# yangao07/longcallD

Measured on AMD Instinct MI355X. Metric: regions_per_sec, higher is better.
Workload: dtype int32; 1 GPU; configs[1]: synthetic 30x hifi region jobs, 10 Mb of reference per step (1250 regions/step, ~20.2 Mbase POA-aligned/step); distinct_batches_per_gpu=32, warmup_on_other_seeds=True, lanes_per_gpu=2

## Files before the change

longcalld_amd/csrc/edlib_kernel.hip:

```cpp
#include <hip/hip_runtime.h>
#include "lcd_types.h"
#include "lcd_kernels.h"

namespace {

typedef unsigned long long Word;

__device__ __forceinline__ int imin(int a, int b) { return a < b ? a : b; }
__device__ __forceinline__ int wave_shr1(const int v) { return __builtin_amdgcn_update_dpp(0, v, 0x138, 0xf, 0xf, false); }

__device__ __forceinline__ int calc_block(Word Pv, Word Mv, Word Eq, int hin, Word &PvOut, Word &MvOut) {
    const Word hinIsNeg = (Word)(hin < 0);
    const Word Xv = Eq | Mv;
    Eq |= hinIsNeg;
    const Word Xh = (((Eq & Pv) + Pv) ^ Pv) | Eq;
    Word Ph = Mv | ~(Xh | Pv);
    Word Mh = Pv & Xh;
    int hout = (int)(Ph >> 63) - (int)(Mh >> 63);
    Ph <<= 1; Mh <<= 1;
    Mh |= hinIsNeg;
    Ph |= (Word)(hin > 0);
    PvOut = Mh | ~(Xv | Ph);
    MvOut = Ph & Xv;
    return hout;
}

struct Sub {
    const uint8_t *q, *t;
    int qlen, tlen;
};

template <bool STORE, bool COLS>
__device__ __forceinline__ int myers_pass(const Sub &sp, int ncols, bool rev, int lane, Word *P, Word *M, int *S, int *col_out, signed char *hcarry,
                                          unsigned long long *blocks_acc) {
    const int qlen = sp.qlen, nb = (qlen + 63) >> 6;
    int result = 0;
    __shared__ uint8_t tbuf[128];
    for (int tile0 = 0; tile0 < nb; tile0 += 64) {
        const int b = tile0 + lane;
        const bool act = b < nb;
        Word peq[5] = {0, 0, 0, 0, 0};
        if (act) {
            const int base = b << 6, lim = imin(64, qlen - base);
            for (int r = 0; r < lim; ++r) {
                const int qi = base + r;
                const uint8_t c = rev ? sp.q[qlen - 1 - qi] : sp.q[qi];
                const Word bit = 1ull << r;
                if (c == 0) peq[0] |= bit; else if (c == 1) peq[1] |= bit; else if (c == 2) peq[2] |= bit;
                else if (c == 3) peq[3] |= bit; else peq[4] |= bit;
            }
        }
        Word Pv = ~0ull, Mv = 0;
        int score = (b + 1) << 6, hout = 0;
        const bool more = tile0 + 64 < nb;
        const int nsteps = ncols + 63;
        auto tchar = [&](const int cc) -> uint8_t { return cc < ncols ? (rev ? sp.t[sp.tlen - 1 - cc] : sp.t[cc]) : (uint8_t)4; };
        uint8_t tnext = tchar(lane);
        int hcnext = (tile0 != 0 && lane < ncols) ? (int)hcarry[lane] : 0, hcreg = 0;
        for (int step = 0; step < nsteps; ++step) {
            if ((step & 63) == 0) {
                const int cc = step + lane;
                __syncthreads();
                tbuf[cc & 127] = tnext;
                hcreg = hcnext;
                __syncthreads();
                tnext = tchar(cc + 64);
                if (tile0 != 0) hcnext = cc + 64 < ncols ? (int)hcarry[cc + 64] : 0;
            }
            const int hleft = wave_shr1(hout);
            const int c = step - lane;
            const int hc0 = __builtin_amdgcn_readlane(hcreg, step & 63);
            if (act && c >= 0 && c < ncols) {
                const int hin = lane == 0 ? (tile0 == 0 ? 1 : hc0) : hleft;
                const uint8_t tc = tbuf[c & 127];
                const Word Eq = tc == 0 ? peq[0] : tc == 1 ? peq[1] : tc == 2 ? peq[2] : tc == 3 ? peq[3] : peq[4];
                hout = calc_block(Pv, Mv, Eq, hin, Pv, Mv);
                score += hout;
                if (STORE) { const size_t o = (size_t)c * nb + b; P[o] = Pv; M[o] = Mv; S[o] = score; }
                if (more && lane == 63) hcarry[ncols + c] = (signed char)hout;
            }
        }
        __syncthreads();
        if (more) {
            for (int c = lane; c < ncols; c += 64) hcarry[c] = hcarry[ncols + c];
            __syncthreads();
        }
        *blocks_acc += (unsigned long long)ncols * (unsigned long long)(imin(64, nb - tile0));
        if (act) {
            const int base = b << 6, lim = imin(64, qlen - base);
            if (COLS)
                for (int pos = 0; pos < lim; ++pos) {
                    int v = score;
                    if (pos < 63) v += -__popcll(Pv >> (pos + 1)) + __popcll(Mv >> (pos + 1));
                    col_out[base + pos] = v;
                }
        }
        const int lastb = nb - 1;
        if (lastb >= tile0 && lastb < tile0 + 64) {
            const int pos = (qlen - 1) & 63;
            int v = score;
            if (pos < 63) v += -__popcll(Pv >> (pos + 1)) + __popcll(Mv >> (pos + 1));
            result = __shfl(v, lastb - tile0);
        }
        __syncthreads();
    }
    return result;
}

template <int HIN0>
__device__ __forceinline__ void sg_pass(const Sub &sp, int ncols, bool rev, int lane, signed char *hcarry, unsigned long long *blocks_acc, int *best_out, int *first_out, int *last_out) {
    const int qlen = sp.qlen, nb = (qlen + 63) >> 6;
    int best = 1 << 30, first_c = -1, last_c = -1;
    __shared__ uint8_t tbuf2[128];
    for (int tile0 = 0; tile0 < nb; tile0 += 64) {
        const int b = tile0 + lane;
        const bool act = b < nb;
        Word peq[5] = {0, 0, 0, 0, 0};
        if (act) {
            const int base = b << 6, lim = imin(64, qlen - base);
            for (int r = 0; r < lim; ++r) {
                const int qi = base + r;
                const uint8_t c = rev ? sp.q[qlen - 1 - qi] : sp.q[qi];
                const Word bit = 1ull << r;
                if (c == 0) peq[0] |= bit; else if (c == 1) peq[1] |= bit; else if (c == 2) peq[2] |= bit;
                else if (c == 3) peq[3] |= bit; else peq[4] |= bit;
            }
        }
        Word Pv = ~0ull, Mv = 0;
        int score = (b + 1) << 6, hout = 0;
        const bool more = tile0 + 64 < nb;
        const bool is_last = b == nb - 1;
        const int pos = (qlen - 1) & 63;
        const int nsteps = ncols + 63;
        auto tchar = [&](const int cc) -> uint8_t { return cc < ncols ? (rev ? sp.t[sp.tlen - 1 - cc] : sp.t[cc]) : (uint8_t)4; };
        uint8_t tnext = tchar(lane);
        int hcnext = (tile0 != 0 && lane < ncols) ? (int)hcarry[lane] : 0, hcreg = 0;
        for (int step = 0; step < nsteps; ++step) {
            if ((step & 63) == 0) {
                const int cc = step + lane;
                __syncthreads();
                tbuf2[cc & 127] = tnext;
                hcreg = hcnext;
                __syncthreads();
                tnext = tchar(cc + 64);
                if (tile0 != 0) hcnext = cc + 64 < ncols ? (int)hcarry[cc + 64] : 0;
            }
            const int hleft = wave_shr1(hout);
            const int c = step - lane;
            const int hc0 = __builtin_amdgcn_readlane(hcreg, step & 63);
            if (act && c >= 0 && c < ncols) {
                const int hin = lane == 0 ? (tile0 == 0 ? HIN0 : hc0) : hleft;
                const uint8_t tc = tbuf2[c & 127];
                const Word Eq = tc == 0 ? peq[0] : tc == 1 ? peq[1] : tc == 2 ? peq[2] : tc == 3 ? peq[3] : peq[4];
                hout = calc_block(Pv, Mv, Eq, hin, Pv, Mv);
                score += hout;
                if (more && lane == 63) hcarry[ncols + c] = (signed char)hout;
                if (is_last) {
                    int v = score;
                    if (pos < 63) v += -__popcll(Pv >> (pos + 1)) + __popcll(Mv >> (pos + 1));
                    if (v < best) { best = v; first_c = c; last_c = c; } else if (v == best) last_c = c;
                }
            }
        }
        __syncthreads();
        if (more) {
            for (int c = lane; c < ncols; c += 64) hcarry[c] = hcarry[ncols + c];
            __syncthreads();
        }
        *blocks_acc += (unsigned long long)ncols * (unsigned long long)(imin(64, nb - tile0));
        const int lastb = nb - 1;
        if (lastb >= tile0 && lastb < tile0 + 64) { best = __shfl(best, lastb - tile0); first_c = __shfl(first_c, lastb - tile0); last_c = __shfl(last_c, lastb - tile0); }
        __syncthreads();
    }
    *best_out = best; *first_out = first_c; *last_out = last_c;
}

struct Tally {
    int n_mis, n_eq, n_ins, n_del, runs;
    int last_op;
};

}

__global__ void __launch_bounds__(64) lcd_edlib_kernel(const EdJob *jobs, const uint8_t *pool, uint8_t *arena, EdOut *outs, int n_jobs) {
    const int jid = blockIdx.x;
    if (jid >= n_jobs) return;
    const int lane = threadIdx.x;
    const EdJob jb = jobs[jid];
    EdOut out; out.status = LCD_OK; out.dist = -1; out.xgaps = 0; out.n_eq = 0; out.n_xid = 0; out.blocks = 0; out.start = 0; out.end = jb.tlen - 1;
    const uint8_t *q = pool + jb.q_off, *t = pool + jb.t_off;
    const int qlen = jb.qlen, tlen = jb.tlen;
    if (qlen == 0 || tlen == 0) {
        out.dist = jb.mode == 1 ? qlen : (qlen > tlen ? qlen : tlen);
        if (jb.mode == 1) { out.start = -1; out.end = -1; }
        if (lane == 0) outs[jb.pad_] = out;
        return;
    }
    const size_t TB_CAP = (size_t)ed_tb_cap(qlen, tlen);
    uint8_t *ws = arena + jb.ws_off;
    Word *P = (Word *)ws, *M = P + TB_CAP;
    int *S = (int *)(M + TB_CAP);
    int *colL = S + TB_CAP, *colR = colL + qlen;
    signed char *hcarry = (signed char *)(colR + qlen);
    unsigned long long blocks = 0;
    Sub top = {q, t, qlen, tlen};
    int dist, t0 = 0, tl0 = tlen;
    const bool top_leaf = jb.mode != 1 && 20ll * ((qlen + 63) >> 6) * tlen + 8ll * tlen < 1024 * 1024;
    if (jb.mode == 1) {
        int best, endf, endl, best2, sf, sl;
        sg_pass<0>(top, tlen, false, lane, hcarry, &blocks, &best, &endf, &endl);
        if (best >= qlen) {
            out.dist = qlen; out.start = 0; out.end = -1;
            out.xgaps = 1; out.n_eq = 0; out.n_xid = qlen; out.blocks = blocks;
            if (lane == 0) outs[jb.pad_] = out;
            return;
        }
        Sub pre = {q, t, qlen, endf + 1};
        sg_pass<1>(pre, endf + 1, true, lane, hcarry, &blocks, &best2, &sf, &sl);
        if (best2 != best || endf < 0 || sl < 0) { out.status = LCD_ERR_BACKTRACK; if (lane == 0) outs[jb.pad_] = out; return; }
        dist = best; t0 = endf - sl; tl0 = sl + 1;
        out.start = t0; out.end = endf;
    } else if (top_leaf)
        dist = -1;
    else
        dist = myers_pass<false, false>(top, tlen, false, lane, nullptr, nullptr, nullptr, nullptr, hcarry, &blocks);
    out.dist = dist;
    __shared__ int stk[64][5];
    int sp = 0;
    if (lane == 0) { stk[0][0] = 0; stk[0][1] = qlen; stk[0][2] = t0; stk[0][3] = tl0; stk[0][4] = dist; }
    sp = 1;
    __syncthreads();
    Tally T = {0, 0, 0, 0, 0, -1};
    while (sp > 0 && out.status == LCD_OK) {
        --sp;
        const int qo = stk[sp][0], ql = stk[sp][1], to = stk[sp][2], tl = stk[sp][3], best = stk[sp][4];
        __syncthreads();
        if (ql == 0 || tl == 0) {
            const int n = ql + tl;
            if (n > 0) {
                const int op = ql == 0 ? 2 : 1;
                if (op == 2) T.n_del += n; else T.n_ins += n;
                if (T.last_op != op) T.runs++;
                T.last_op = op;
            }
            continue;
        }
        Sub s = {q + qo, t + to, ql, tl};
        const long long nb = (ql + 63) >> 6;
        const long long data_size = 20ll * nb * tl + 8ll * tl;
        if (data_size < 1024 * 1024) {
            const int leaf_score = myers_pass<true, false>(s, tl, false, lane, P, M, S, nullptr, hcarry, &blocks);
            if (top_leaf) out.dist = leaf_score;
            __syncthreads();
            int r_mis = 0, r_eq = 0, r_ins = 0, r_del = 0, r_runs = 0, leaf_first = -1, leaf_last = -1;
            {
                const int NB = (int)nb;
                int c0 = -1, bA = -1;
                Word cPa = 0, cMa = 0, cPb = 0, cMb = 0; int cSa = 0, cSb = 0;
                auto refresh = [&](const int r, const int c) {
                    c0 = c; bA = r >> 6;
                    const int cl = c - lane;
                    if (cl >= 0) {
                        const size_t oa = (size_t)cl * NB + bA;
                        cPa = P[oa]; cMa = M[oa]; cSa = S[oa];
                        if (bA > 0) { cPb = P[oa - 1]; cMb = M[oa - 1]; cSb = S[oa - 1]; }
                    }
                };
                auto rl64 = [&](const Word v, const int l) { return (Word)(unsigned)__builtin_amdgcn_readlane((int)(unsigned)v, l) | ((Word)(unsigned)__builtin_amdgcn_readlane((int)(unsigned)(v >> 32), l) << 32); };
                auto val = [&](const int r, const int c) -> int {
                    if (r < 0) return c + 1;
                    if (c < 0) return r + 1;
                    const int b = r >> 6, l = __builtin_amdgcn_readfirstlane(c0 - c), pos = r & 63;
                    Word pv, mv; int sv;
                    if (l >= 0 && l < 64 && b == bA) { pv = rl64(cPa, l); mv = rl64(cMa, l); sv = __builtin_amdgcn_readlane(cSa, l); }
                    else if (l >= 0 && l < 64 && b == bA - 1) { pv = rl64(cPb, l); mv = rl64(cMb, l); sv = __builtin_amdgcn_readlane(cSb, l); }
                    else { const size_t o = (size_t)c * NB + b; pv = P[o]; mv = M[o]; sv = S[o]; }
                    return sv + (pos < 63 ? (-__popcll(pv >> (pos + 1)) + __popcll(mv >> (pos + 1))) : 0);
                };
                int r = __builtin_amdgcn_readfirstlane(ql - 1), c = __builtin_amdgcn_readfirstlane(tl - 1), prev = -1;
                refresh(r, c);
                int cur = val(r, c);
                auto vbit = [&](const Word wa, const Word wb, const Word *G, const int r, const int c) -> int {
                    const int b = r >> 6, l = __builtin_amdgcn_readfirstlane(c0 - c), pos = r & 63;
                    unsigned h;
                    if (l >= 0 && l < 64 && (b == bA || b == bA - 1)) { const Word w = b == bA ? wa : wb; h = (unsigned)__builtin_amdgcn_readlane((int)(unsigned)(pos < 32 ? w : w >> 32), l); }
                    else { const Word w = G[(size_t)c * NB + b]; h = (unsigned)(pos < 32 ? w : w >> 32); }
                    return (int)((h >> (pos & 31)) & 1u);
                };
                while (r >= 0 && c >= 0) {
                    if (c - 1 < c0 - 63 || (r > 0 && ((r - 1) >> 6) < bA - 1)) refresh(r, c);
                    int op;
                    if (vbit(cPa, cPb, P, r, c)) { op = 1; --r; cur -= 1; }
                    else {
                        const int left = val(r, c - 1);
                        if (left + 1 == cur) { op = 2; --c; cur = left; }
                        else {
                            const int d = c == 0 ? val(r - 1, c - 1) : left - vbit(cPa, cPb, P, r, c - 1) + vbit(cMa, cMb, M, r, c - 1);
                            op = d == cur ? 0 : 3; --r; --c; cur = d;
                        }
                    }
                    r = __builtin_amdgcn_readfirstlane(r); c = __builtin_amdgcn_readfirstlane(c); cur = __builtin_amdgcn_readfirstlane(cur);
                    if (op == 0) r_eq++; else if (op == 3) r_mis++; else { if (op == 1) r_ins++; else r_del++; if (op != prev) r_runs++; }
                    if (leaf_last < 0) leaf_last = op;
                    leaf_first = op; prev = op;
                }
                if (c >= 0) { const int n = c + 1; r_del += n; if (prev != 2) r_runs++; if (leaf_last < 0) leaf_last = 2; leaf_first = 2; }
                if (r >= 0) { const int n = r + 1; r_ins += n; if (prev != 1) r_runs++; if (leaf_last < 0) leaf_last = 1; leaf_first = 1; }
            }
            T.n_mis += r_mis; T.n_eq += r_eq; T.n_ins += r_ins; T.n_del += r_del; T.runs += r_runs;
            if (leaf_first >= 0) {
                if ((leaf_first == 1 || leaf_first == 2) && T.last_op == leaf_first) T.runs--;
                T.last_op = leaf_last;
            }
            __syncthreads();
        } else {
            const int left_w = tl / 2, right_w = tl - left_w;
            myers_pass<false, true>(s, left_w, false, lane, nullptr, nullptr, nullptr, colL, hcarry, &blocks);
            myers_pass<false, true>(s, right_w, true, lane, nullptr, nullptr, nullptr, colR, hcarry, &blocks);
            __syncthreads();
            int cand = 1 << 30;
            for (int i = lane; i <= ql - 2; i += 64)
                if (colL[i] + colR[ql - 1 - (i + 1)] == best) { cand = i; break; }
            for (int d = 32; d >= 1; d >>= 1) cand = imin(cand, __shfl_xor(cand, d));
            int q_idx, ls, rs;
            if (cand < (1 << 30)) { q_idx = cand; ls = colL[cand]; rs = colR[ql - 1 - (cand + 1)]; }
            else if (left_w + colR[ql - 1] == best) { q_idx = -1; ls = left_w; rs = colR[ql - 1]; }
            else if (colL[ql - 1] + right_w == best) { q_idx = ql - 1; ls = colL[ql - 1]; rs = right_w; }
            else { out.status = LCD_ERR_BACKTRACK; break; }
            const int ul_h = q_idx + 1, lr_h = ql - ul_h;
            if (sp + 2 > 64) { out.status = LCD_ERR_BACKTRACK; break; }
            __syncthreads();
            if (lane == 0) {
                stk[sp][0] = qo + ul_h; stk[sp][1] = lr_h; stk[sp][2] = to + left_w; stk[sp][3] = right_w; stk[sp][4] = rs;
                stk[sp + 1][0] = qo; stk[sp + 1][1] = ul_h; stk[sp + 1][2] = to; stk[sp + 1][3] = left_w; stk[sp + 1][4] = ls;
            }
            sp += 2;
            __syncthreads();
        }
    }
    out.xgaps = T.n_mis + T.runs;
    out.n_eq = T.n_eq;
    out.n_xid = T.n_mis + T.n_ins + T.n_del;
    out.blocks = blocks;
    if (lane == 0) outs[jb.pad_] = out;
}

void lcd_launch_edlib(const EdJob *jobs, const uint8_t *pool, uint8_t *arena, EdOut *outs, int n_jobs, hipStream_t stream) {
    if (n_jobs <= 0) return;
    hipLaunchKernelGGL(lcd_edlib_kernel, dim3(n_jobs), dim3(64), 0, stream, jobs, pool, arena, outs, n_jobs);
}
```

Baseline: 169,600 regions/s.

## Restructure Myers sweep into chunked wave-synchronous loop with LDS Peq lookup

Merges the global and semi-global Myers passes into one templated sweep that walks 64-step chunks. It replaces per-chunk __syncthreads with wavefront-scope fences and keeps the Peq masks in LDS, indexed directly by the text character instead of a select chain. Steady-state chunks skip the per-lane boundary guards, and the next Eq and text character are software-prefetched. The semi-global pass now tracks the score for the last row incrementally through an hrow bit instead of doing popcounts every step. This cuts sync, branch and ALU overhead in the inner loop, but relies on single-wave workgroup ordering and adds code size and register pressure.

```diff
diff --git a/longcalld_amd/csrc/edlib_kernel.hip b/longcalld_amd/csrc/edlib_kernel.hip
--- a/longcalld_amd/csrc/edlib_kernel.hip
+++ b/longcalld_amd/csrc/edlib_kernel.hip
@@ -9,14 +9,16 @@
 __device__ __forceinline__ int imin(int a, int b) { return a < b ? a : b; }
 __device__ __forceinline__ int wave_shr1(const int v) { return __builtin_amdgcn_update_dpp(0, v, 0x138, 0xf, 0xf, false); }
 
-__device__ __forceinline__ int calc_block(Word Pv, Word Mv, Word Eq, int hin, Word &PvOut, Word &MvOut) {
-    const Word hinIsNeg = (Word)(hin < 0);
+template <bool SG>
+__device__ __forceinline__ int calc_block(Word Pv, Word Mv, Word Eq, int hin, Word &PvOut, Word &MvOut, int pos, int &hrow) {
+    const Word hinIsNeg = (Word)((unsigned)hin >> 31);
     const Word Xv = Eq | Mv;
     Eq |= hinIsNeg;
     const Word Xh = (((Eq & Pv) + Pv) ^ Pv) | Eq;
     Word Ph = Mv | ~(Xh | Pv);
     Word Mh = Pv & Xh;
     int hout = (int)(Ph >> 63) - (int)(Mh >> 63);
+    if (SG) hrow = (int)((unsigned)(Ph >> pos) & 1u) - (int)((unsigned)(Mh >> pos) & 1u);
     Ph <<= 1; Mh <<= 1;
     Mh |= hinIsNeg;
     Ph |= (Word)(hin > 0);
@@ -30,12 +32,60 @@
     int qlen, tlen;
 };
 
-template <bool STORE, bool COLS>
-__device__ __forceinline__ int myers_pass(const Sub &sp, int ncols, bool rev, int lane, Word *P, Word *M, int *S, int *col_out, signed char *hcarry,
-                                          unsigned long long *blocks_acc) {
+struct SweepLds { Word eq[5][64]; uint8_t ring[128]; };
+
+__device__ __forceinline__ void lds_wave_order() { __builtin_amdgcn_fence(__ATOMIC_RELEASE, "wavefront"); __builtin_amdgcn_wave_barrier(); __builtin_amdgcn_fence(__ATOMIC_ACQUIRE, "wavefront"); }
+__device__ __forceinline__ void mem_wave_order() { __builtin_amdgcn_fence(__ATOMIC_SEQ_CST, "workgroup"); __builtin_amdgcn_wave_barrier(); }
+
+template <bool STORE, bool SG>
+struct Sweep {
+    SweepLds *L;
+    int lane, ncols, b, nb, pos, h0;
+    bool act, more;
+    Word Pv, Mv; int score, hout;
+    int best, first_c, last_c;
+    Word *P, *M; int *S;
+    signed char *hcarry;
+    int hcreg;
+    template <bool SINGLE, bool GUARD>
+    __device__ __forceinline__ void run(const int s0, const int n) {
+        const unsigned lane8 = (unsigned)lane << 3;
+        const char *eqb = (const char *)&L->eq[0][0];
+        unsigned tc_n = L->ring[(s0 - lane) & 127];
+        Word eq_n = *(const Word *)(eqb + (tc_n << 9) + lane8);
+        tc_n = L->ring[(s0 + 1 - lane) & 127];
+        unsigned o8 = STORE ? (unsigned)((s0 - lane) * nb + b) << 3 : 0u;
+        const unsigned nb8 = (unsigned)nb << 3;
+        for (int i = 0; i < n; ++i) {
+            const int c = s0 + i - lane;
+            const Word Eq = eq_n;
+            eq_n = *(const Word *)(eqb + (tc_n << 9) + lane8);
+            tc_n = L->ring[(c + 2) & 127];
+            const int hl0 = SINGLE ? h0 : __builtin_amdgcn_readlane(hcreg, i);
+            const int hin = __builtin_amdgcn_update_dpp(hl0, hout, 0x138, 0xf, 0xf, false);
+            if (!GUARD || (act && c >= 0 && c < ncols)) {
+                int hrow = 0;
+                hout = calc_block<SG>(Pv, Mv, Eq, hin, Pv, Mv, pos, hrow);
+                score += SG ? hrow : hout;
+                if (STORE) if (GUARD || act) { *(Word *)((char *)P + o8) = Pv; *(Word *)((char *)M + o8) = Mv; *(int *)((char *)S + (o8 >> 1)) = score; }
+                if (!SINGLE) if (more && lane == 63) hcarry[ncols + c] = (signed char)hout;
+                if (SG) {
+                    const bool lt = score < best, le = score <= best;
+                    best = lt ? score : best; first_c = lt ? c : first_c; last_c = le ? c : last_c;
+                }
+            }
+            if (STORE) o8 += nb8;
+            asm volatile("" : "+v"(eq_n), "+v"(tc_n));
+        }
+    }
+};
+
+template <bool STORE, bool COLS, bool SG, int H0>
+__device__ __forceinline__ int sweep_pass(SweepLds *L, const Sub &sp, int ncols, bool rev, int lane, Word *P, Word *M, int *S, int *col_out, signed char *hcarry,
+                                          unsigned long long *blocks_acc, int *best_out, int *first_out, int *last_out) {
     const int qlen = sp.qlen, nb = (qlen + 63) >> 6;
     int result = 0;
-    __shared__ uint8_t tbuf[128];
+    int best = 1 << 30, first_c = -1, last_c = -1;
     for (int tile0 = 0; tile0 < nb; tile0 += 64) {
         const int b = tile0 + lane;
         const bool act = b < nb;
@@ -50,129 +100,73 @@
                 else if (c == 3) peq[3] |= bit; else peq[4] |= bit;
             }
         }
-        Word Pv = ~0ull, Mv = 0;
-        int score = (b + 1) << 6, hout = 0;
         const bool more = tile0 + 64 < nb;
+        const bool single = tile0 == 0 && !more;
         const int nsteps = ncols + 63;
-        auto tchar = [&](const int cc) -> uint8_t { return cc < ncols ? (rev ? sp.t[sp.tlen - 1 - cc] : sp.t[cc]) : (uint8_t)4; };
+        Sweep<STORE, SG> W;
+        W.L = L; W.lane = lane; W.ncols = ncols; W.b = b; W.nb = nb; W.pos = (qlen - 1) & 63; W.h0 = H0; W.act = act; W.more = more;
+        W.Pv = ~0ull; W.Mv = 0; W.hout = 0;
+        W.score = SG ? (b << 6) + W.pos + 1 : (b + 1) << 6;
+        W.best = 1 << 30; W.first_c = -1; W.last_c = -1;
+        W.P = P; W.M = M; W.S = S; W.hcarry = hcarry; W.hcreg = 0;
+        lds_wave_order();
+        for (int k = 0; k < 5; ++k) L->eq[k][lane] = peq[k];
+        L->ring[lane] = 4; L->ring[lane + 64] = 4;
+        auto tchar = [&](const int cc) -> uint8_t { if (cc >= ncols) return (uint8_t)4; const uint8_t ch = rev ? sp.t[sp.tlen - 1 - cc] : sp.t[cc]; return ch < 4 ? ch : (uint8_t)4; };
         uint8_t tnext = tchar(lane);
-        int hcnext = (tile0 != 0 && lane < ncols) ? (int)hcarry[lane] : 0, hcreg = 0;
-        for (int step = 0; step < nsteps; ++step) {
-            if ((step & 63) == 0) {
-                const int cc = step + lane;
-                __syncthreads();
-                tbuf[cc & 127] = tnext;
-                hcreg = hcnext;
-                __syncthreads();
-                tnext = tchar(cc + 64);
-                if (tile0 != 0) hcnext = cc + 64 < ncols ? (int)hcarry[cc + 64] : 0;
-            }
-            const int hleft = wave_shr1(hout);
-            const int c = step - lane;
-            const int hc0 = __builtin_amdgcn_readlane(hcreg, step & 63);
-            if (act && c >= 0 && c < ncols) {
-                const int hin = lane == 0 ? (tile0 == 0 ? 1 : hc0) : hleft;
-                const uint8_t tc = tbuf[c & 127];
-                const Word Eq = tc == 0 ? peq[0] : tc == 1 ? peq[1] : tc == 2 ? peq[2] : tc == 3 ? peq[3] : peq[4];
-                hout = calc_block(Pv, Mv, Eq, hin, Pv, Mv);
-                score += hout;
-                if (STORE) { const size_t o = (size_t)c * nb + b; P[o] = Pv; M[o] = Mv; S[o] = score; }
-                if (more && lane == 63) hcarry[ncols + c] = (signed char)hout;
-            }
-        }
-        __syncthreads();
+        int hcnext = tile0 == 0 ? H0 : (lane < ncols ? (int)hcarry[lane] : 0);
+        for (int s0 = 0; s0 < nsteps; s0 += 64) {
+            const int cc = s0 + lane;
+            lds_wave_order();
+            L->ring[cc & 127] = tnext;
+            W.hcreg = hcnext;
+            lds_wave_order();
+            tnext = tchar(cc + 64);
+            if (tile0 != 0) hcnext = cc + 64 < ncols ? (int)hcarry[cc + 64] : 0;
+            const int n = imin(64, nsteps - s0);
+            const bool steady = s0 >= 64 && s0 + 63 < ncols;
+            if (single) { if (steady) W.template run<true, false>(s0, 64); else W.template run<true, true>(s0, n); }
+            else { if (steady) W.template run<false, false>(s0, 64); else W.template run<false, true>(s0, n); }
+        }
+        mem_wave_order();
         if (more) {
             for (int c = lane; c < ncols; c += 64) hcarry[c] = hcarry[ncols + c];
-            __syncthreads();
+            mem_wave_order();
         }
         *blocks_acc += (unsigned long long)ncols * (unsigned long long)(imin(64, nb - tile0));
-        if (act) {
-            const int base = b << 6, lim = imin(64, qlen - base);
-            if (COLS)
+        const int lastb = nb - 1;
+        if (SG) {
+            if (lastb >= tile0 && lastb < tile0 + 64) { best = __shfl(W.best, lastb - tile0); first_c = __shfl(W.first_c, lastb - tile0); last_c = __shfl(W.last_c, lastb - tile0); }
+        } else {
+            if (COLS && act) {
+                const int base = b << 6, lim = imin(64, qlen - base);
                 for (int pos = 0; pos < lim; ++pos) {
-                    int v = score;
-                    if (pos < 63) v += -__popcll(Pv >> (pos + 1)) + __popcll(Mv >> (pos + 1));
+                    int v = W.score;
+                    if (pos < 63) v += -__popcll(W.Pv >> (pos + 1)) + __popcll(W.Mv >> (pos + 1));
                     col_out[base + pos] = v;
                 }
-        }
-        const int lastb = nb - 1;
-        if (lastb >= tile0 && lastb < tile0 + 64) {
-            const int pos = (qlen - 1) & 63;
-            int v = score;
-            if (pos < 63) v += -__popcll(Pv >> (pos + 1)) + __popcll(Mv >> (pos + 1));
-            result = __shfl(v, lastb - tile0);
-        }
-        __syncthreads();
+            }
+            if (lastb >= tile0 && lastb < tile0 + 64) {
+                const int pos = (qlen - 1) & 63;
+                int v = W.score;
+                if (pos < 63) v += -__popcll(W.Pv >> (pos + 1)) + __popcll(W.Mv >> (pos + 1));
+                result = __shfl(v, lastb - tile0);
+            }
+        }
+        mem_wave_order();
     }
+    if (SG) { *best_out = best; *first_out = first_c; *last_out = last_c; }
     return result;
 }
 
+template <bool STORE, bool COLS>
+__device__ __forceinline__ int myers_pass(SweepLds *L, const Sub &sp, int ncols, bool rev, int lane, Word *P, Word *M, int *S, int *col_out, signed char *hcarry,
+                                          unsigned long long *blocks_acc) {
+    return sweep_pass<STORE, COLS, false, 1>(L, sp, ncols, rev, lane, P, M, S, col_out, hcarry, blocks_acc, nullptr, nullptr, nullptr);
+}
 template <int HIN0>
-__device__ __forceinline__ void sg_pass(const Sub &sp, int ncols, bool rev, int lane, signed char *hcarry, unsigned long long *blocks_acc, int *best_out, int *first_out, int *last_out) {
-    const int qlen = sp.qlen, nb = (qlen + 63) >> 6;
-    int best = 1 << 30, first_c = -1, last_c = -1;
-    __shared__ uint8_t tbuf2[128];
-    for (int tile0 = 0; tile0 < nb; tile0 += 64) {
-        const int b = tile0 + lane;
-        const bool act = b < nb;
-        Word peq[5] = {0, 0, 0, 0, 0};
-        if (act) {
-            const int base = b << 6, lim = imin(64, qlen - base);
-            for (int r = 0; r < lim; ++r) {
-                const int qi = base + r;
-                const uint8_t c = rev ? sp.q[qlen - 1 - qi] : sp.q[qi];
-                const Word bit = 1ull << r;
-                if (c == 0) peq[0] |= bit; else if (c == 1) peq[1] |= bit; else if (c == 2) peq[2] |= bit;
-                else if (c == 3) peq[3] |= bit; else peq[4] |= bit;
-            }
-        }
-        Word Pv = ~0ull, Mv = 0;
-        int score = (b + 1) << 6, hout = 0;
-        const bool more = tile0 + 64 < nb;
-        const bool is_last = b == nb - 1;
-        const int pos = (qlen - 1) & 63;
-        const int nsteps = ncols + 63;
-        auto tchar = [&](const int cc) -> uint8_t { return cc < ncols ? (rev ? sp.t[sp.tlen - 1 - cc] : sp.t[cc]) : (uint8_t)4; };
-        uint8_t tnext = tchar(lane);
-        int hcnext = (tile0 != 0 && lane < ncols) ? (int)hcarry[lane] : 0, hcreg = 0;
-        for (int step = 0; step < nsteps; ++step) {
-            if ((step & 63) == 0) {
-                const int cc = step + lane;
-                __syncthreads();
-                tbuf2[cc & 127] = tnext;
-                hcreg = hcnext;
-                __syncthreads();
-                tnext = tchar(cc + 64);
-                if (tile0 != 0) hcnext = cc + 64 < ncols ? (int)hcarry[cc + 64] : 0;
-            }
-            const int hleft = wave_shr1(hout);
-            const int c = step - lane;
-            const int hc0 = __builtin_amdgcn_readlane(hcreg, step & 63);
-            if (act && c >= 0 && c < ncols) {
-                const int hin = lane == 0 ? (tile0 == 0 ? HIN0 : hc0) : hleft;
-                const uint8_t tc = tbuf2[c & 127];
-                const Word Eq = tc == 0 ? peq[0] : tc == 1 ? peq[1] : tc == 2 ? peq[2] : tc == 3 ? peq[3] : peq[4];
-                hout = calc_block(Pv, Mv, Eq, hin, Pv, Mv);
-                score += hout;
-                if (more && lane == 63) hcarry[ncols + c] = (signed char)hout;
-                if (is_last) {
-                    int v = score;
-                    if (pos < 63) v += -__popcll(Pv >> (pos + 1)) + __popcll(Mv >> (pos + 1));
-                    if (v < best) { best = v; first_c = c; last_c = c; } else if (v == best) last_c = c;
-                }
-            }
-        }
-        __syncthreads();
-        if (more) {
-            for (int c = lane; c < ncols; c += 64) hcarry[c] = hcarry[ncols + c];
-            __syncthreads();
-        }
-        *blocks_acc += (unsigned long long)ncols * (unsigned long long)(imin(64, nb - tile0));
-        const int lastb = nb - 1;
-        if (lastb >= tile0 && lastb < tile0 + 64) { best = __shfl(best, lastb - tile0); first_c = __shfl(first_c, lastb - tile0); last_c = __shfl(last_c, lastb - tile0); }
-        __syncthreads();
-    }
-    *best_out = best; *first_out = first_c; *last_out = last_c;
+__device__ __forceinline__ void sg_pass(SweepLds *L, const Sub &sp, int ncols, bool rev, int lane, signed char *hcarry, unsigned long long *blocks_acc, int *best_out, int *first_out, int *last_out) {
+    sweep_pass<false, false, true, HIN0>(L, sp, ncols, rev, lane, nullptr, nullptr, nullptr, nullptr, hcarry, blocks_acc, best_out, first_out, last_out);
 }
 
 struct Tally {
@@ -203,12 +197,13 @@
     int *colL = S + TB_CAP, *colR = colL + qlen;
     signed char *hcarry = (signed char *)(colR + qlen);
     unsigned long long blocks = 0;
+    __shared__ SweepLds sweep_lds;
     Sub top = {q, t, qlen, tlen};
     int dist, t0 = 0, tl0 = tlen;
     const bool top_leaf = jb.mode != 1 && 20ll * ((qlen + 63) >> 6) * tlen + 8ll * tlen < 1024 * 1024;
     if (jb.mode == 1) {
         int best, endf, endl, best2, sf, sl;
-        sg_pass<0>(top, tlen, false, lane, hcarry, &blocks, &best, &endf, &endl);
+        sg_pass<0>(&sweep_lds, top, tlen, false, lane, hcarry, &blocks, &best, &endf, &endl);
         if (best >= qlen) {
             out.dist = qlen; out.start = 0; out.end = -1;
             out.xgaps = 1; out.n_eq = 0; out.n_xid = qlen; out.blocks = blocks;
@@ -216,14 +211,14 @@
             return;
         }
         Sub pre = {q, t, qlen, endf + 1};
-        sg_pass<1>(pre, endf + 1, true, lane, hcarry, &blocks, &best2, &sf, &sl);
+        sg_pass<1>(&sweep_lds, pre, endf + 1, true, lane, hcarry, &blocks, &best2, &sf, &sl);
         if (best2 != best || endf < 0 || sl < 0) { out.status = LCD_ERR_BACKTRACK; if (lane == 0) outs[jb.pad_] = out; return; }
         dist = best; t0 = endf - sl; tl0 = sl + 1;
         out.start = t0; out.end = endf;
     } else if (top_leaf)
         dist = -1;
     else
-        dist = myers_pass<false, false>(top, tlen, false, lane, nullptr, nullptr, nullptr, nullptr, hcarry, &blocks);
+        dist = myers_pass<false, false>(&sweep_lds, top, tlen, false, lane, nullptr, nullptr, nullptr, nullptr, hcarry, &blocks);
     out.dist = dist;
     __shared__ int stk[64][5];
     int sp = 0;
@@ -249,7 +244,7 @@
         const long long nb = (ql + 63) >> 6;
         const long long data_size = 20ll * nb * tl + 8ll * tl;
         if (data_size < 1024 * 1024) {
-            const int leaf_score = myers_pass<true, false>(s, tl, false, lane, P, M, S, nullptr, hcarry, &blocks);
+            const int leaf_score = myers_pass<true, false>(&sweep_lds, s, tl, false, lane, P, M, S, nullptr, hcarry, &blocks);
             if (top_leaf) out.dist = leaf_score;
             __syncthreads();
             int r_mis = 0, r_eq = 0, r_ins = 0, r_del = 0, r_runs = 0, leaf_first = -1, leaf_last = -1;
@@ -315,8 +310,8 @@
             __syncthreads();
         } else {
             const int left_w = tl / 2, right_w = tl - left_w;
-            myers_pass<false, true>(s, left_w, false, lane, nullptr, nullptr, nullptr, colL, hcarry, &blocks);
-            myers_pass<false, true>(s, right_w, true, lane, nullptr, nullptr, nullptr, colR, hcarry, &blocks);
+            myers_pass<false, true>(&sweep_lds, s, left_w, false, lane, nullptr, nullptr, nullptr, colL, hcarry, &blocks);
+            myers_pass<false, true>(&sweep_lds, s, right_w, true, lane, nullptr, nullptr, nullptr, colR, hcarry, &blocks);
             __syncthreads();
             int cand = 1 << 30;
             for (int i = lane; i <= ql - 2; i += 64)
```

Measured after the change: 168,600 regions/s. About the same (-0.6%).
